# HiLab-git/FPL-plus

Hardware: AMD Instinct MI355X
Metric: 3D volumes/sec (train step, 80x160x160) (higher is better)
Workload: dtype bf16; 1 GPU; UNet3D-DSBN 32-base-ch bf16 (fp32 master weights), per-GPU batch 2x1x80x160x160 synthetic VS crops, DiceLoss + Adam, domain alternating per step; global_batch=2, parallelism=dp1, step=zero_grad+forward+loss+backward+allreduce+adam

## Files before the change

fpl-plus_amd/csrc/common.h:

```cpp
#pragma once
#include <hip/hip_runtime.h>
#include <math.h>
#include <stdint.h>
#include <stdio.h>
#include <stdarg.h>
#include <string.h>
#include "../../include/fplx.h"

typedef __bf16 bf16_t;

#define FPLX_WAVE 64

inline char* fplx_err_buf() {
  static thread_local char buf[512];
  return buf;
}
inline int fplx_fail(int code, const char* fmt, ...) {
  va_list ap;
  va_start(ap, fmt);
  vsnprintf(fplx_err_buf(), 512, fmt, ap);
  va_end(ap);
  return code;
}
inline int fplx_check_launch(const char* what) {
// ... 221 lines not shown
  t.step = (gridDim.x - c + 7u) >> 3;
  return t;
}
template <typename... P, typename... A>
inline void fplx_launch(void (*kernel)(P...), dim3 grid, dim3 block, size_t lds, hipStream_t st, A... args) {
  if (lds) (void)hipFuncSetAttribute((const void*)kernel, hipFuncAttributeMaxDynamicSharedMemorySize, (int)lds);
  kernel<<<grid, block, lds, st>>>(args...);
}
#endif
#define FPLX_KNOB_LIST(X)                                                                                              \
  X(XCD, "xcd", 1)                                                    \
  X(BRICK, "brick", 1)                                    \
  X(BRICK_FILL, "brick_fill", 192)           \
  X(BRICK_GEO, "brick_geo", -1)                    \
  X(BRICK_KSPLIT, "brick_ksplit", 0)                                             \
  X(EDGE_BLOCKS, "edge_blocks", 1024)                             \
  X(STEM_ROWS, "stem_rows", 1)                                              \
  X(OUTCONV_T, "outconv_t", 1)                                 \
  X(OUTCONV_DGRAD_MFMA, "outconv_dgrad_mfma", 1)                                                                       \
  X(OUTCONV_FWD_ROWS, "outconv_fwd_rows", 1)  \
  X(OUTCONV_DGRAD_ROWS, "outconv_dgrad_rows", 1)  \
  X(PACK_TILED, "pack_tiled", 1)                                                                                       \
  X(PACK_MULTI, "pack_multi", 1)                                                                                       \
  X(MARCH, "march", 1)                           \
  X(MARCH64_FW, "march64_fw", 0)                                \
  X(MARCH_DS, "march_ds", 0)                                       \
  X(MARCH128, "march128", 1)                                                                                           \
  X(MARCH64_LW, "march64_lw", 1)            \
  X(MARCH32_V2, "march32_v2", 4)              \
  X(WG_COT_MINVOX, "wg_cot_minvox", 0)                                                                                 \
  X(WG_TW, "wg_tw", 0)                                                                                                 \
  X(WG_CIT, "wg_cit", 2)                                                                                               \
  X(WG_COT, "wg_cot", 2)                                                                                               \
  X(WG_DS, "wg_ds", 0)                                                                                                 \
  X(WG_VOX, "wg_vox", 1)                              \
  X(WG_ROLL, "wg_roll", 1)                     \
  X(WG_ROLL_GEO, "wg_roll_geo", 0)          \
  X(WG_ROLL_M16, "wg_roll_m16", 1)                 \
  X(WG_ROLL_MB, "wg_roll_mb", 1)            \
  X(WG_ROLL_CUS, "wg_roll_cus", 256)                                \
  X(WG_ROLL_OVH, "wg_roll_ovh", 9)                     \
  X(WG_ROLL_MINVOX, "wg_roll_minvox", 0)                                                   \
  X(WG_ROLL2D, "wg_roll2d", 1)              \
  X(WG_ROLL2D_OVH, "wg_roll2d_ovh", 3)      \
  X(WG_REDUCE_ROWS, "wg_reduce_rows", 8)    \
  X(WG_VOX_LW, "wg_vox_lw", 1)              \
  X(WG_VOX_CUS, "wg_vox_cus", 128)          \
  X(WG_VOX_MAXV, "wg_vox_maxv", 10000)         \
  X(TILE_NT, "tile_nt", 0)                                                                                             \
  X(TILE_KS, "tile_ks", 0)                                                                                             \
  X(MID_TILE, "mid_tile", 1)                                                                                           \
  X(DECONV_ROWS, "deconv_rows", 1)                                                                                     \
  X(DECONV_DGRAD_ROWS, "deconv_dgrad_rows", 1)   \
  X(ROWS_SMALL_DIV, "rows_small_div", 16)   \
  X(EW_GROUP, "ew_group", 1)                                                                                           \
  X(POOL_COL, "pool_col", 1)                         \
  X(EW_INFLIGHT, "ew_inflight", 2)          \
  X(EW_INFLIGHT_REDUCE, "ew_inflight_reduce", 2)
enum FplxKnobId {
#define FPLX_KNOB_ENUM(id, key, def) FPLX_K_##id,
  FPLX_KNOB_LIST(FPLX_KNOB_ENUM)
#undef FPLX_KNOB_ENUM
  FPLX_K_COUNT
};
extern "C" __attribute__((visibility("hidden"))) int64_t fplx_knob_values[FPLX_K_COUNT];
static inline int64_t fplx_knob(int id) { return __atomic_load_n(&fplx_knob_values[id], __ATOMIC_RELAXED); }
static inline int fplx_xcd_on() { return (int)fplx_knob(FPLX_K_XCD); }

static inline int fplx_rows_for(int64_t voxels) {
  constexpr int cap = 512;
  const int div = voxels <= 32768 ? (int)fplx_knob(FPLX_K_ROWS_SMALL_DIV) : 64;
  int64_t r = (voxels + div - 1) / div;
  if (r > cap) r = cap;
  if (r < 1) r = 1;
  return (int)r;
}
```

fpl-plus_amd/csrc/conv_generic.hip:

```cpp
#include "internal.h"

namespace {

struct Strides { int64_t n, d, h, w, c; };

constexpr int CO_T = 8;
constexpr int FWD_THREADS = 256;
constexpr int MAX_ROWS = 2048;

template <typename TX, typename TW, typename TY>
__global__ void __launch_bounds__(FWD_THREADS)
conv_fwd_generic(const TX* __restrict__ x, Strides xs, const TW* __restrict__ wp, const float* __restrict__ bias,
                 TY* __restrict__ y, Strides ys, int N, int D, int H, int W, int Cin, int Cout,
                 int KD, int KH, int KW, float* __restrict__ stats, int64_t tiles) {
  const int co0 = blockIdx.y * CO_T;
  const int64_t V = (int64_t)N * D * H * W;
  float s[CO_T], q[CO_T];
#pragma unroll
  for (int j = 0; j < CO_T; ++j) s[j] = q[j] = 0.f;
  const int pd = KD / 2, ph = KH / 2, pw = KW / 2;
  for (int64_t tile = blockIdx.x; tile < tiles; tile += gridDim.x) {
    const int64_t v = tile * FWD_THREADS + threadIdx.x;
    const bool valid = v < V;
    int64_t r = valid ? v : 0;
// ... 1214 lines not shown
  Strides xs{(int64_t)d * h * w * ldx, (int64_t)h * w * ldx, (int64_t)w * ldx, ldx, 1};
  Strides ys{(int64_t)4 * sd * d * h * w * ldy, (int64_t)(sd == 2 ? 4 : 2) * h * w * ldy, (int64_t)2 * w * ldy, ldy, 1};
  bool done = false;
  if (dt == FPLX_BF16) {
    const size_t m = fplx_mfma_deconv2_wgrad_ws_bytes(n, d, h, w, cin, cout);
    if (m > 0) {
      int r = fplx_mfma_deconv2_wgrad(x, ldx, dy, ldy, dw, db, n, d, h, w, cin, cout, ws, m, sd, st);
      if (r < 0) return r;
      if (r == 1) { done = true; used = m; db = nullptr; }
    }
  }
  float* bpart = (float*)((char*)ws + used);
  if (done) {
  } else if (dt == FPLX_F32)
    wgrad_generic<float, float, true><<<grid, WG_THREADS, 0, st>>>((const float*)x, xs, (const float*)dy, ys, part, n,
                                                                   d, h, w, cin, cout, sd, 2, 2, chunks);
  else if (dt == FPLX_BF16)
    wgrad_generic<bf16_t, bf16_t, true><<<grid, WG_THREADS, 0, st>>>((const bf16_t*)x, xs, (const bf16_t*)dy, ys, part,
                                                                     n, d, h, w, cin, cout, sd, 2, 2, chunks);
  else
    return fplx_fail(FPLX_E_BADDTYPE, "deconv2_wgrad: dtype %d", dt);
  if (!done) wgrad_reduce<<<grid_for((int64_t)taps * cout * cin, 256, 1024), 256, 0, st>>>(part, dw, chunks, taps, cout, cin, 1);
  if (db) {
    Strides yb{(int64_t)4 * sd * d * h * w * ldy, (int64_t)4 * h * w * ldy, (int64_t)2 * w * ldy, ldy, 1};
    if (dt == FPLX_F32) launch_bias_grad<float>((const float*)dy, yb, n, sd * d, 2 * h, 2 * w, cout, bpart, db, st);
    else launch_bias_grad<bf16_t>((const bf16_t*)dy, yb, n, sd * d, 2 * h, 2 * w, cout, bpart, db, st);
  }
  return fplx_check_launch("deconv2_wgrad");
}

int fplx_deconv2_fwd(const void* x, int64_t ldx, const void* wf, const float* bias, void* y, int64_t ldy, int n, int d,
                     int h, int w, int cin, int cout, int dt, fplx_stream_t stream) {
  return deconv_fwd_impl(x, ldx, wf, bias, y, ldy, n, d, h, w, cin, cout, dt, 2, stream);
}
int fplx_deconv2_dgrad(const void* dy, int64_t ldy, const void* wb, void* dx, int64_t ldx, int n, int d, int h, int w,
                       int cin, int cout, int dt, fplx_stream_t stream) {
  return deconv_dgrad_impl(dy, ldy, wb, dx, ldx, n, d, h, w, cin, cout, dt, 2, stream);
}
size_t fplx_deconv2_wgrad_ws_bytes(int n, int d, int h, int w, int cin, int cout) {
  return deconv_wgrad_ws_impl(n, d, h, w, cin, cout, 2);
}
int fplx_deconv2_wgrad(const void* x, int64_t ldx, const void* dy, int64_t ldy, float* dw, float* db, int n, int d,
                       int h, int w, int cin, int cout, int dt, void* ws, size_t ws_bytes, fplx_stream_t stream) {
  return deconv_wgrad_impl(x, ldx, dy, ldy, dw, db, n, d, h, w, cin, cout, dt, ws, ws_bytes, 2, stream);
}
int fplx_deconv122_fwd(const void* x, int64_t ldx, const void* wf, const float* bias, void* y, int64_t ldy, int n, int d,
                       int h, int w, int cin, int cout, int dt, fplx_stream_t stream) {
  return deconv_fwd_impl(x, ldx, wf, bias, y, ldy, n, d, h, w, cin, cout, dt, 1, stream);
}
int fplx_deconv122_dgrad(const void* dy, int64_t ldy, const void* wb, void* dx, int64_t ldx, int n, int d, int h, int w,
                         int cin, int cout, int dt, fplx_stream_t stream) {
  return deconv_dgrad_impl(dy, ldy, wb, dx, ldx, n, d, h, w, cin, cout, dt, 1, stream);
}
size_t fplx_deconv122_wgrad_ws_bytes(int n, int d, int h, int w, int cin, int cout) {
  return deconv_wgrad_ws_impl(n, d, h, w, cin, cout, 1);
}
int fplx_deconv122_wgrad(const void* x, int64_t ldx, const void* dy, int64_t ldy, float* dw, float* db, int n, int d,
                         int h, int w, int cin, int cout, int dt, void* ws, size_t ws_bytes, fplx_stream_t stream) {
  return deconv_wgrad_impl(x, ldx, dy, ldy, dw, db, n, d, h, w, cin, cout, dt, ws, ws_bytes, 1, stream);
}

}
```

fpl-plus_amd/csrc/conv_mfma.hip:

```cpp
#include "internal.h"
#include "gfx950.h"
#include <stdlib.h>

namespace {

constexpr int DIRECT_THREADS = 256;

template <int MT, int NTL, int MODE>
__global__ void __launch_bounds__(DIRECT_THREADS)
conv_fwd_direct(const bf16_t* __restrict__ x, int64_t ldx, const bf16_t* __restrict__ wp,
                const float* __restrict__ bias, bf16_t* __restrict__ y, int64_t ldy, int N, int D, int H, int W,
                int Cin, int Cout, float* __restrict__ stats, float* __restrict__ partial = nullptr) {
  const int lane = threadIdx.x & 63, wave = threadIdx.x >> 6;
  const int r = lane & 31, kh8 = (lane >> 5) * 8;
  const int64_t V = (int64_t)N * D * H * W;
  const int64_t m0 = ((int64_t)blockIdx.x * 4 + wave) * (MT * 32);
  const int n0 = blockIdx.y * (NTL * 32);

  int vn[MT], vd[MT], vh[MT], vw[MT];
  bool vok[MT];
#pragma unroll
  for (int t = 0; t < MT; ++t) {
    int64_t v = m0 + t * 32 + r;
    vok[t] = v < V;
// ... 1198 lines not shown
    __syncthreads();
    if (tid < 32) {
      const int cc = tid >> 3, j = tid & 7;
      float t = 0.f;
      for (int k = 0; k < 64; ++k) t += red[(k * 4 + cc) * 8 + j];
      bpart[(int64_t)blockIdx.x * Cout + cot * 32 + tid] = t;
    }
  }
}

__global__ void __launch_bounds__(64) deconv_bias_reduce(const float* __restrict__ bpart, int rows, int C, float* __restrict__ db) {
  const int c = blockIdx.x;
  float t = 0.f;
  for (int r = threadIdx.x; r < rows; r += 64) t += bpart[(int64_t)r * C + c];
  t = wave_sum(t);
  if (threadIdx.x == 0) db[c] = t;
}

__global__ void __launch_bounds__(256)
deconv_wgrad_reduce(const float* __restrict__ part, int nblk, int npairs, int cit, int Cin, int Cout,
                    float* __restrict__ dw, int ntaps) {
  __shared__ float red[256];
  const int64_t per = (int64_t)8 * cit * 1024, total = npairs * per;
  const int64_t i = (int64_t)blockIdx.x * 64 + (threadIdx.x & 63);
  const int pl = threadIdx.x >> 6, o = threadIdx.x & 63;
  float t = 0.f;
  if (i < total)
    for (int b = pl; b < nblk; b += 4) t += part[(int64_t)b * total + i];
  red[pl * 64 + o] = t;
  __syncthreads();
  if (pl != 0 || i >= total) return;
  t = red[o] + red[64 + o] + red[128 + o] + red[192 + o];
  const int co_l = i & 31, ci_l = (i >> 5) & 31, c = (int)((i >> 10) % cit), tap = (int)((i / (1024 * cit)) % 8);
  const int pair = (int)(i / per);
  const int ncig = Cin / (32 * cit);
  const int co = (pair / ncig) * 32 + co_l, ci = ((pair % ncig) * cit + c) * 32 + ci_l;
  if (tap < ntaps) dw[((int64_t)ci * Cout + co) * ntaps + tap] = t;
}

struct DwCfg { int cit, npairs, nblk; size_t ws; };
inline DwCfg dw_cfg(int n, int d, int h, int w, int cin, int cout) {
  DwCfg c;
  c.cit = (cin % 128 == 0) ? 4 : (cin % 64 == 0 ? 2 : 1);
  c.npairs = (cin / (32 * c.cit)) * (cout / 32);
  const int64_t chunks = ((int64_t)n * d * h * w + 127) / 128;
  int nb = 512 / c.npairs;
  if (nb < 1) nb = 1;
  if (nb > chunks) nb = (int)chunks;
  c.nblk = nb;
  c.ws = (size_t)c.nblk * c.npairs * 8 * c.cit * 1024 * sizeof(float) + (size_t)c.nblk * cout * sizeof(float);
  return c;
}

template <int NT, int KC>
__global__ void __launch_bounds__(256, 2)
conv_fwd_tile(const bf16_t* __restrict__ x, int64_t ldx, const bf16_t* __restrict__ wp, const float* __restrict__ bias,
              bf16_t* __restrict__ y, int64_t ldy, int N, int D, int H, int W, int Cin, int Cout,
              float* __restrict__ stats, float* __restrict__ partial, int tap_lo, int tap_cnt, int xcd) {
  constexpr int MTL = 128, THREADS = MTL * 2, NTW = NT / 64;
  constexpr int ROWB = KC * 2, CH = KC / 8, RP = THREADS / CH;
  constexpr int PA = MTL / RP, PB = NT / RP;
  constexpr int KS = KC / 16;
  constexpr int A_BYTES = MTL * ROWB, B_BYTES = NT * ROWB, BUF = A_BYTES + B_BYTES;
  extern __shared__ __attribute__((aligned(16))) char smem[];
  const int tid = threadIdx.x, lane = tid & 63, wave = tid >> 6;
  const int r = lane & 31, khalf = lane >> 5;
  const int wm = wave >> 1, wn = wave & 1;
  const int64_t V = (int64_t)N * D * H * W;
  const FplxBlock bid = fplx_xcd_block(xcd);
  const int64_t m0 = (int64_t)bid.x * MTL;
  const int n0 = bid.y * NT;
  const int c16 = tid % CH, row0 = tid / CH;
  const bf16_t* abase[PA];
  uint32_t amask[PA];
#pragma unroll
  for (int u = 0; u < PA; ++u) {
    int64_t v = m0 + row0 + RP * u;
    const bool ok = v < V;
    if (!ok) v = 0;
    abase[u] = x + v * ldx + c16 * 8;
    unsigned q = (unsigned)v;
    const int ww0 = (int)(q % (unsigned)W); q /= (unsigned)W;
    const int hh0 = (int)(q % (unsigned)H); q /= (unsigned)H;
    const int dd0 = (int)(q % (unsigned)D);
    uint32_t m = 0;
    for (int t = 0; t < 27; ++t) {
      const int dd = dd0 + t / 9 - 1, hh = hh0 + (t / 3) % 3 - 1, ww = ww0 + t % 3 - 1;
      if (ok && dd >= 0 && dd < D && hh >= 0 && hh < H && ww >= 0 && ww < W) m |= 1u << t;
    }
    amask[u] = m;
  }
  const int nkc = Cin / KC;
  const int ntaps = (tap_cnt - bid.z + (int)gridDim.z - 1) / (int)gridDim.z;
  const int niter = ntaps * nkc;
  auto swz = [](int row) { return (row / (16 / CH)) % CH; };
  uint4 areg00, areg01, areg02, areg03, breg00, breg01, breg02, breg03;
  uint4 areg10, areg11, areg12, areg13, breg10, breg11, breg12, breg13;
  areg02 = areg03 = breg01 = breg02 = breg03 = make_uint4(0, 0, 0, 0);
  areg12 = areg13 = breg11 = breg12 = breg13 = make_uint4(0, 0, 0, 0);
  unsigned zmask0 = 0, zmask1 = 0;
#define TILE_A(U, S)                                                                                                \
  if (PA > (U)) {                                                                                                   \
    constexpr int u_ = (U) < PA ? (U) : 0;                                                                          \
    const bool in_ = (amask[u_] >> tap_) & 1u;                                                                      \
    zmask##S |= in_ ? 0u : (1u << (U));                                                                             \
    areg##S##U = *reinterpret_cast<const uint4*>(abase[u_] + (in_ ? aoff_ : (int64_t)kc_));                         \
// ... 644 lines not shown
      int rc = fplx_check_launch("mfma_deconv2_fwd_rows");
      return rc < 0 ? rc : 1;
    }
  }
  dim3 grid((unsigned)((V + 127) / 128), cout / 32, sd);
  deconv_fwd_mfma<<<grid, DIRECT_THREADS, 0, st>>>((const bf16_t*)x, ldx, (const bf16_t*)wf, bias, (bf16_t*)y, ldy, n, d,
                                                   h, w, cin, cout, sd, vec_ok, fplx_xcd_on());
  int rc = fplx_check_launch("mfma_deconv2_fwd");
  return rc < 0 ? rc : 1;
}

extern "C" int fplx_mfma_deconv2_dgrad(const void* dy, int64_t ldy, const void* wb, void* dx, int64_t ldx, int n, int d,
                                       int h, int w, int cin, int cout, int sd, hipStream_t st) {
  if (cout % 16 != 0 || cin % 32 != 0 || ldy % 8 != 0 || ((uintptr_t)dy % 16) || ((uintptr_t)wb % 16)) return 0;
  const int64_t V = (int64_t)n * d * h * w;
  if (V * 8 >= ((int64_t)1 << 31)) return 0;
  if (sd == 2 && fplx_knob(FPLX_K_DECONV_DGRAD_ROWS) && V >= 16 * 1024 && ldx % 8 == 0 && ((uintptr_t)dx % 16) == 0 &&
      ((cout == 32 && cin == 64) || (cout == 64 && cin == 128))) {
    const int mb = cin == 64 ? 64 : 32;
    const int segsW = (w + mb - 1) / mb;
    const int64_t nseg = (int64_t)n * d * h * segsW;
    const unsigned nb = (unsigned)(nseg < 512 ? nseg : 512);
    if (cout == 32)
      deconv_dgrad_rows<1, 2><<<nb, 256, 0, st>>>((const bf16_t*)dy, ldy, (const bf16_t*)wb, (bf16_t*)dx, ldx, n, d, h, w, segsW, nseg, fplx_xcd_on());
    else
      deconv_dgrad_rows<2, 4><<<nb, 256, 0, st>>>((const bf16_t*)dy, ldy, (const bf16_t*)wb, (bf16_t*)dx, ldx, n, d, h, w, segsW, nseg, fplx_xcd_on());
    int rcr = fplx_check_launch("mfma_deconv2_dgrad_rows");
    return rcr < 0 ? rcr : 1;
  }
  if (sd == 2 && fplx_knob(FPLX_K_DECONV_DGRAD_ROWS) && ((V + 127) / 128) * (cin / 64) < 128 && cin % 64 == 0 && cout % 16 == 0 &&
      ldx % 8 == 0 && ((uintptr_t)dx % 16) == 0) {
    dim3 gs((unsigned)((V + 31) / 32), cin / 64);
    deconv_dgrad_small<<<gs, 256, 0, st>>>((const bf16_t*)dy, ldy, (const bf16_t*)wb, (bf16_t*)dx, ldx, n, d, h, w, cout, cin);
    int rcs = fplx_check_launch("mfma_deconv2_dgrad_small");
    return rcs < 0 ? rcs : 1;
  }
  const bool wide = cin % 64 == 0;
  const dim3 grid = wide ? dim3((unsigned)((V + 255) / 256), cin / 64) : dim3((unsigned)((V + 511) / 512), cin / 32);
  const bool deep = wide && (int64_t)grid.x * grid.y < 192;
  const auto k = deep ? (sd == 2 ? conv_fwd_direct<1, 2, 1> : conv_fwd_direct<1, 2, 2>)
                 : wide ? (sd == 2 ? conv_fwd_direct<2, 2, 1> : conv_fwd_direct<2, 2, 2>)
                        : (sd == 2 ? conv_fwd_direct<4, 1, 1> : conv_fwd_direct<4, 1, 2>);
  fplx_launch(k, deep ? dim3((unsigned)((V + 127) / 128), cin / 64) : grid, DIRECT_THREADS, 0, st, (const bf16_t*)dy, ldy,
              (const bf16_t*)wb, nullptr, (bf16_t*)dx, ldx, n, d, h, w, cout, cin, nullptr, nullptr);
  int rc = fplx_check_launch("mfma_deconv2_dgrad");
  return rc < 0 ? rc : 1;
}

extern "C" size_t fplx_mfma_deconv2_wgrad_ws_bytes(int n, int d, int h, int w, int cin, int cout) {
  if (cin % 32 != 0 || cout % 32 != 0) return 0;
  return dw_cfg(n, d, h, w, cin, cout).ws;
}

extern "C" int fplx_mfma_deconv2_wgrad(const void* x, int64_t ldx, const void* dy, int64_t ldy, float* dw, float* db,
                                       int n, int d, int h, int w, int cin, int cout, void* ws, size_t ws_bytes,
                                       int sd, hipStream_t st) {
  if (cin % 32 != 0 || cout % 32 != 0 || ldx % 8 != 0 || ldy % 8 != 0 || ((uintptr_t)x % 16) || ((uintptr_t)dy % 16))
    return 0;
  const DwCfg c = dw_cfg(n, d, h, w, cin, cout);
  if (ws_bytes < c.ws) return fplx_fail(FPLX_E_WORKSPACE, "mfma_deconv2_wgrad: workspace %zu < %zu", ws_bytes, c.ws);
  const size_t lds = (size_t)(c.cit + 8) * 128 * 64;
  float* bpart = db ? (float*)((char*)ws + (size_t)c.nblk * c.npairs * 8 * c.cit * 1024 * sizeof(float)) : nullptr;
  auto launch = [&](auto kernel) {
    fplx_launch(kernel, dim3(c.nblk, c.npairs), 256, lds, st, (const bf16_t*)x, ldx, (const bf16_t*)dy, ldy, (float*)ws, bpart, n, d,
                h, w, cin, cout, sd);
  };
  if (c.cit == 4) launch(deconv_wgrad_mfma<4>);
  else if (c.cit == 2) launch(deconv_wgrad_mfma<2>);
  else launch(deconv_wgrad_mfma<1>);
  const int64_t total = (int64_t)c.npairs * 8 * c.cit * 1024;
  if (db) deconv_bias_reduce<<<cout, 64, 0, st>>>(bpart, c.nblk, cout, db);
  deconv_wgrad_reduce<<<(unsigned)((total + 63) / 64), 256, 0, st>>>((const float*)ws, c.nblk, c.npairs, c.cit, cin, cout, dw,
                                                                      4 * sd);
  int rc = fplx_check_launch("mfma_deconv2_wgrad");
  return rc < 0 ? rc : 1;
}
```

fpl-plus_amd/csrc/internal.h:

```cpp
#pragma once
#include "common.h"

extern "C" {

int fplx_march_ok(int n, int d, int h, int w, int cin, int cout);
int fplx_march_rows(int n, int d, int h, int w, int cin, int cout);
int fplx_march_variant(int n, int d, int h, int w, int cin, int cout);
int fplx_march_conv3d_fwd(const void* x, int64_t ldx, const void* wp, const float* bias, void* y, int64_t ldy, int n, int d,
                          int h, int w, int cin, int cout, float* stats, hipStream_t st, const void* x1, void* y1, int twod);
int fplx_march_conv3d_fwd_act(const void* x, int64_t ldx, const void* wp, const float* bias, void* y, int64_t ldy, int n,
                              int d, int h, int w, int cin, int cout, float* stats, hipStream_t st, const void* x1, void* y1,
                              int twod, const float* slope, int nmod0);

int fplx_brick_ok(int n, int d, int h, int w, int cin, int cout);
int fplx_brick_first(int n, int d, int h, int w, int cin, int cout);
int fplx_brick_plan(int n, int d, int h, int w, int cin, int cout, int* geo, int* ksplit, int* bricks);
int fplx_brick_conv3d_fwd_act(const void* x, int64_t ldx, const void* wp, const float* bias, void* y, int64_t ldy, int n,
                              int d, int h, int w, int cin, int cout, float* stats, float* partial, int geo, int ksplit,
                              hipStream_t st, const float* slope, const void* x1, int nmod0);

int fplx_wgroll_ok(int n, int d, int h, int w, int cin, int cout, int mid, int splitx);
size_t fplx_wgroll_ws_bytes(int n, int d, int h, int w, int cin, int cout);
int fplx_wgroll_conv3d_wgrad(const void* x, int64_t ldx, const void* dy, int64_t ldy, float* dw, int n, int d, int h, int w,
                             int cin, int cout, void* ws, size_t ws_bytes, hipStream_t st, const void* x1, int mid);

int fplx_mfma_conv3d_plan(int n, int d, int h, int w, int cin, int cout, int mid, int* kernel, int* geo, int* ksplit);
int fplx_mfma_conv3d_stats_rows(int n, int d, int h, int w, int cin, int cout, int mid);
size_t fplx_mfma_conv3d_fwd_ws_bytes(int n, int d, int h, int w, int cin, int cout, int mid);
int fplx_mfma_conv3d_fwd(const void* x, int64_t ldx, const void* wp, const float* bias, void* y, int64_t ldy, int n, int d,
                         int h, int w, int cin, int cout, float* stats, void* ws, size_t ws_bytes, int mid, hipStream_t st);
int fplx_mfma_conv3d_act_ok(int n, int d, int h, int w, int cin, int cout, int mid);
int fplx_mfma_conv3d_act_cat2_ok(int n, int d, int h, int w, int cin, int cout, int mid);
int fplx_mfma_conv3d_fwd_act(const void* x, int64_t ldx, const void* wp, const float* bias, const float* slope, void* y,
                             int64_t ldy, int n, int d, int h, int w, int cin, int cout, void* ws, size_t ws_bytes, int mid,
                             hipStream_t st);
int fplx_mfma_conv3d_fwd_act_cat2(const void* x0, const void* x1, int64_t ldx, const void* wp, const float* bias,
                                  const float* slope, void* y, int64_t ldy, int n, int d, int h, int w, int cin, int cout,
                                  int nmod0, hipStream_t st);
int fplx_mfma_conv3d_wgrad_cit(int n, int d, int h, int w, int cin, int cout);
size_t fplx_mfma_conv3d_wgrad_ws_bytes(int n, int d, int h, int w, int cin, int cout);
int fplx_mfma_conv3d_wgrad(const void* x, int64_t ldx, const void* dy, int64_t ldy, float* dw, int n, int d, int h, int w,
                           int cin, int cout, void* ws, size_t ws_bytes, hipStream_t st, const void* x1, int mid);
int fplx_wgrad_reduce_launch(const float* part, int nblk, int npairs, int cin, int cout, float* dw, int mid, hipStream_t st);
int fplx_mfma_deconv2_fwd(const void* x, int64_t ldx, const void* wf, const float* bias, void* y, int64_t ldy, int n, int d,
                          int h, int w, int cin, int cout, int sd, hipStream_t st);
int fplx_mfma_deconv2_dgrad(const void* dy, int64_t ldy, const void* wb, void* dx, int64_t ldx, int n, int d, int h, int w,
                            int cin, int cout, int sd, hipStream_t st);
size_t fplx_mfma_deconv2_wgrad_ws_bytes(int n, int d, int h, int w, int cin, int cout);
int fplx_mfma_deconv2_wgrad(const void* x, int64_t ldx, const void* dy, int64_t ldy, float* dw, float* db, int n, int d,
                            int h, int w, int cin, int cout, void* ws, size_t ws_bytes, int sd, hipStream_t st);

int fplx_edge_stem_rows(int n, int d, int h, int w, int cin, int cout);
int fplx_edge_stem_fwd(const float* x, const void* wf, const float* bias, void* y, int64_t ldy, int n, int d, int h, int w,
                       int cin, int cout, float* stats, hipStream_t st);
size_t fplx_edge_stem_wgrad_ws_bytes(int n, int d, int h, int w, int cin, int cout);
int fplx_edge_stem_wgrad(const float* x, const void* dy, int64_t ldy, float* dw, int n, int d, int h, int w, int cin,
                         int cout, void* ws, hipStream_t st);
int fplx_edge_stem_wgrad_bn(const float* x, const void* dy, int64_t ldy, float* dw, int n, int d, int h, int w, int cin,
                            int cout, void* ws, hipStream_t st, const void* y, int64_t ldyy, const float* mean,
                            const float* rstd, const float* scale, const float* shift, const float* slope, const float* coef);
int fplx_edge_outconv_fwd(const void* x, int64_t ldx, const float* wf, const float* bias, float* out, int n, int d, int h,
                          int w, int cin, int ncls, hipStream_t st);
int fplx_edge_outconv_dgrad(const float* dl, const void* wb, void* dx, int64_t ldx, int n, int d, int h, int w, int c0,
                            int ncls, hipStream_t st);
size_t fplx_edge_outconv_wgrad_ws_bytes(int n, int d, int h, int w, int c0, int ncls);
int fplx_edge_outconv_wgrad(const void* x, int64_t ldx, const float* dl, float* dw, int n, int d, int h, int w, int c0,
                            int ncls, void* ws, hipStream_t st);
int fplx_edge_outconv_bn_ok(int n, int d, int h, int w, int c0, int ncls);
int fplx_edge_outconv_bn_rows(int n, int d, int h, int w, int ncls);
int fplx_edge_outconv_fwd_bn(const void* y, int64_t ldy, const float* scale, const float* shift, const float* slope, void* a,
                             int64_t lda, const float* wf, const float* bias, float* out, int n, int d, int h, int w, int c0,
                             int ncls, hipStream_t st);
int fplx_edge_outconv_dgrad_bn(int mode, const float* dl, const void* wb, const void* y, int64_t ldy, const float* mean,
                               const float* rstd, const float* scale, const float* shift, const float* slope,
                               const float* coef, float* part, void* dy, int64_t lddy, int n, int d, int h, int w, int c0,
                               int ncls, hipStream_t st);
size_t fplx_edge_outconv_wgrad_bn_ws_bytes(int n, int d, int h, int w, int c0, int ncls);
int fplx_edge_outconv_wgrad_bn(const void* y, int64_t ldy, const float* scale, const float* shift, const float* slope,
                               const float* dl, float* dw, float* db, int n, int d, int h, int w, int c0, int ncls, void* ws,
                               hipStream_t st);

}
```

fpl-plus_amd/fplx/ops.py:

```python
import ctypes
import math

import numpy as np
import torch
from . import _lib
from ._lib import F32, BF16, call

_DT = {torch.float32: F32, torch.bfloat16: BF16}


def dt_of(t):
    try:
        return _DT[t.dtype]
    except KeyError:
        raise ValueError("fplx: unsupported activation dtype {0:}".format(t.dtype))


def ptr(t):
    return 0 if t is None else t.data_ptr()


def stream():
    return torch.cuda.current_stream().cuda_stream

# ... 159 lines not shown
    call("fplx_conv2d_fwd_cat2" if mid else "fplx_conv3d_fwd_cat2", ptr(x0), ptr(x1), ld_of(x0), ptr(wp), ptr(bias), ptr(y), ld_of(y), n, d, h, w, cin,
         cout, ptr(stats), stream())


def conv3d_dgrad_split2(dy, wb, dx0, dx1, dims, cin, cout, mid=False):
    n, d, h, w = dims
    assert ld_of(dx0) == ld_of(dx1)
    call("fplx_conv2d_dgrad_split2" if mid else "fplx_conv3d_dgrad_split2", ptr(dy), ld_of(dy), ptr(wb), ptr(dx0), ptr(dx1), ld_of(dx0), n, d, h, w, cin,
         cout, stream())


def conv3d_wgrad_cat2(x0, x1, dy, dw, dims, cin, cout, ws, mid=False):
    n, d, h, w = dims
    assert ld_of(x0) == ld_of(x1)
    call("fplx_conv2d_wgrad_cat2" if mid else "fplx_conv3d_wgrad_cat2", ptr(x0), ptr(x1), ld_of(x0), ptr(dy), ld_of(dy),
         ptr(dw), n, d, h, w, cin, cout, ptr(ws), ws.numel() * ws.element_size(), stream())


def conv3d_fwd_act_ok(dims, cin, cout, mid=False, cat2=False):
    n, d, h, w = dims
    return _lib.lib().fplx_conv3d_fwd_act_ok(n, d, h, w, cin, cout, 1 if mid else 0, 1 if cat2 else 0) == 1


def conv3d_fwd_act(x0, x1, wp, bias, slope, y, dims, cin, cout, mid=False, n_x0=0):
    n, d, h, w = dims
    ws = _fwd_scratch(conv3d_fwd_ws_bytes(dims, cin, cout, (3, 3, 3), BF16, BF16, mid), y.device)
    if x1 is not None:
        assert ld_of(x0) == ld_of(x1)
    call("fplx_conv3d_fwd_act", ptr(x0), ptr(x1), ld_of(x0), ptr(wp), ptr(bias), ptr(slope), ptr(y), ld_of(y), n, d, h, w, cin,
         cout, 1 if mid else 0, int(n_x0), ptr(ws), 0 if ws is None else ws.numel(), stream())


def _dc(sd):
    return "fplx_deconv2_" if sd == 2 else "fplx_deconv122_"


def deconv2_fwd(x, wf, bias, y, dims, cin, cout, sd=2):
    n, d, h, w = dims
    call(_dc(sd) + "fwd", ptr(x), ld_of(x), ptr(wf), ptr(bias), ptr(y), ld_of(y), n, d, h, w, cin, cout,
         dt_of(x), stream())


def deconv2_dgrad(dy, wb, dx, dims, cin, cout, sd=2):
    n, d, h, w = dims
    call(_dc(sd) + "dgrad", ptr(dy), ld_of(dy), ptr(wb), ptr(dx), ld_of(dx), n, d, h, w, cin, cout,
         dt_of(dy), stream())


def deconv2_wgrad_ws_bytes(dims, cin, cout, sd=2):
    n, d, h, w = dims
    return getattr(_lib.lib(), _dc(sd) + "wgrad_ws_bytes")(n, d, h, w, cin, cout)


def deconv2_wgrad(x, dy, dw, db, dims, cin, cout, ws, sd=2):
    n, d, h, w = dims
    call(_dc(sd) + "wgrad", ptr(x), ld_of(x), ptr(dy), ld_of(dy), ptr(dw), ptr(db), n, d, h, w, cin, cout,
         dt_of(x), ptr(ws), ws.numel() * ws.element_size(), stream())


def upsample2_fwd(x, y, dims, c, sd=2):
    n, d, h, w = dims
    call("fplx_upsample2_fwd", ptr(x), ld_of(x), ptr(y), ld_of(y), n, d, h, w, c, dt_of(x), sd, stream())


def upsample2_bwd(dy, dx, dims, c, sd=2):
    n, d, h, w = dims
    call("fplx_upsample2_bwd", ptr(dy), ld_of(dy), ptr(dx), ld_of(dx), n, d, h, w, c, dt_of(dy), sd, stream())


def bn_train_finalize(stats, rows, c, count, gamma, beta, rm, rv, nbt, bnbuf, momentum=0.1, eps=1e-5):
    call("fplx_bn_train_finalize", ptr(stats), rows, c, count, ptr(gamma), ptr(beta), ptr(rm), ptr(rv), ptr(nbt),
         momentum, eps, ptr(bnbuf[0]), ptr(bnbuf[1]), ptr(bnbuf[2]), ptr(bnbuf[3]), stream())


def bn_eval_prepare(gamma, beta, rm, rv, bnbuf, eps=1e-5):
    c = gamma.numel()
    call("fplx_bn_eval_prepare", ptr(gamma), ptr(beta), ptr(rm), ptr(rv), eps, c, ptr(bnbuf[2]), ptr(bnbuf[3]),
         stream())


def bn_act_fwd(y, out, bnbuf, slope, p, seed, sid, c):
    call("fplx_bn_act_fwd", ptr(y), ld_of(y), ptr(out), ld_of(out), ptr(bnbuf[2]), ptr(bnbuf[3]), ptr(slope),
         float(p), int(seed), int(sid), y.shape[0], c, dt_of(y), stream())


def num_partials(voxels):
    return _lib.lib().fplx_num_partials(voxels)


def outconv_bn_rows(dims, c0=32, ncls=2):
    n, d, h, w = dims
    return _lib.lib().fplx_outconv_bn_rows(n, d, h, w, int(c0), int(ncls))


def outconv_bn_ok(dims, c0, ncls):
    return outconv_bn_rows(dims, c0, ncls) > 0


def outconv_fwd_bn(y, bnbuf, slope, a, wf, bias, logits, dims, c0, ncls):
    n, d, h, w = dims
    call("fplx_outconv_fwd_bn", ptr(y), ld_of(y), ptr(bnbuf[2]), ptr(bnbuf[3]), ptr(slope), ptr(a), int(c0) if a is None else ld_of(a),
         ptr(wf), ptr(bias), ptr(logits), n, d, h, w, int(c0), int(ncls), stream())


def outconv_wgrad_bn_ws_bytes(dims, c0, ncls):
    n, d, h, w = dims
# ... 1152 lines not shown
```

include/fplx.h:

```cpp
#ifndef FPLX_H
#define FPLX_H

#include <stddef.h>
#include <stdint.h>

#ifdef __cplusplus
extern "C" {
#endif
#pragma GCC visibility push(default)

typedef void* fplx_stream_t;

enum { FPLX_F32 = 0, FPLX_BF16 = 1 };

enum {
  FPLX_OK = 0,
  FPLX_E_BADSHAPE = -1,
  FPLX_E_BADDTYPE = -2,
  FPLX_E_WORKSPACE = -3,
  FPLX_E_HIP = -4,
  FPLX_E_NULL = -5
};

int fplx_version(void);
// ... 9 lines not shown
int fplx_tuning_key(int index, char* buf, size_t n);
int fplx_conv3d_plan_query(int n, int d, int h, int w, int cin, int cout, int kd, int kh, int kw, int x_dt, int y_dt,
                           int* kernel, int* geometry, int* ksplit, int* stats_rows);

int fplx_pack_conv_weight(const float* w, void* wf, void* wb, int cout, int cin, int kd, int kh, int kw,
                          int dt, fplx_stream_t stream);
int fplx_pack_conv_weights_batched(int n, const float* const* w, void* const* wf, void* const* wb, const int* cout,
                                   const int* cin, int dt, float* const* stamp, int verify, fplx_stream_t stream);
int fplx_pack_weights_multi(int n, const int* kind, const float* const* w, void* const* wf, void* const* wb, const int* a,
                            const int* b, const int* taps, const int* dt, fplx_stream_t stream);
int fplx_pack_deconv_weight(const float* w, void* wf, void* wb, int cin, int cout, int dt,
                            fplx_stream_t stream);

int fplx_conv3d_stats_rows(int n, int d, int h, int w, int cin, int cout, int kd, int kh, int kw, int x_dt, int y_dt);
size_t fplx_conv3d_fwd_ws_bytes(int n, int d, int h, int w, int cin, int cout, int kd, int kh, int kw, int x_dt, int y_dt);
int fplx_conv3d_fwd(const void* x, int x_dt, int64_t sn, int64_t sd, int64_t sh, int64_t sw, int64_t sc,
                    const void* wp, const float* bias,
                    void* y, int y_dt, int64_t yn, int64_t yd, int64_t yh, int64_t yw, int64_t yc,
                    int n, int d, int h, int w, int cin, int cout, int kd, int kh, int kw,
                    float* stats, void* ws, size_t ws_bytes, fplx_stream_t stream);

size_t fplx_conv3d_wgrad_ws_bytes(int n, int d, int h, int w, int cin, int cout, int kd, int kh, int kw);
int fplx_conv3d_wgrad(const void* x, int x_dt, int64_t sn, int64_t sd, int64_t sh, int64_t sw, int64_t sc,
                      const void* dy, int dy_dt, int64_t yn, int64_t yd, int64_t yh, int64_t yw, int64_t yc,
                      float* dw, float* db, int n, int d, int h, int w, int cin, int cout,
                      int kd, int kh, int kw, void* ws, size_t ws_bytes, fplx_stream_t stream);

int fplx_stem_wgrad_bn(const float* x, const void* y, int64_t ldy, const void* dout, int64_t ldd, const float* mean,
                       const float* rstd, const float* scale, const float* shift, const float* slope, const float* coef,
                       float* dw, int n, int d, int h, int w, int cin, int cout, void* ws, size_t ws_bytes, fplx_stream_t stream);

int fplx_conv3d_cat2_ok(int n, int d, int h, int w, int cin, int cout);
int fplx_conv3d_fwd_cat2(const void* x0, const void* x1, int64_t ldx, const void* wp, const float* bias, void* y,
                         int64_t ldy, int n, int d, int h, int w, int cin, int cout, float* stats,
                         fplx_stream_t stream);
int fplx_conv3d_dgrad_split2(const void* dy, int64_t ldy, const void* wb, void* dx0, void* dx1, int64_t ldx, int n,
                             int d, int h, int w, int cin, int cout, fplx_stream_t stream);
int fplx_conv3d_wgrad_cat2(const void* x0, const void* x1, int64_t ldx, const void* dy, int64_t ldy, float* dw, int n,
                           int d, int h, int w, int cin, int cout, void* ws, size_t ws_bytes, fplx_stream_t stream);

int fplx_conv3d_fwd_act_ok(int n, int d, int h, int w, int cin, int cout, int mid, int cat2);
int fplx_conv3d_fwd_act(const void* x0, const void* x1, int64_t ldx, const void* wp, const float* bias,
                        const float* prelu_slope, void* y, int64_t ldy, int n, int d, int h, int w, int cin, int cout,
                        int mid, int n_x0, void* ws, size_t ws_bytes, fplx_stream_t stream);

int fplx_deconv2_fwd(const void* x, int64_t ldx, const void* wf, const float* bias, void* y, int64_t ldy,
                     int n, int d, int h, int w, int cin, int cout, int dt, fplx_stream_t stream);
int fplx_deconv2_dgrad(const void* dy, int64_t ldy, const void* wb, void* dx, int64_t ldx,
                       int n, int d, int h, int w, int cin, int cout, int dt, fplx_stream_t stream);
size_t fplx_deconv2_wgrad_ws_bytes(int n, int d, int h, int w, int cin, int cout);
int fplx_deconv2_wgrad(const void* x, int64_t ldx, const void* dy, int64_t ldy, float* dw, float* db,
                       int n, int d, int h, int w, int cin, int cout, int dt,
                       void* ws, size_t ws_bytes, fplx_stream_t stream);

int fplx_pack_conv2d_weight(const float* w, void* wf, void* wb, int cout, int cin, int dt, fplx_stream_t stream);
int fplx_conv2d_stats_rows(int n, int d, int h, int w, int cin, int cout, int x_dt, int y_dt);
size_t fplx_conv2d_fwd_ws_bytes(int n, int d, int h, int w, int cin, int cout, int x_dt, int y_dt);
int fplx_conv2d_fwd(const void* x, int x_dt, int64_t sn, int64_t sd, int64_t sh, int64_t sw, int64_t sc,
                    const void* wp, const float* bias, void* y, int y_dt, int64_t yn, int64_t yd, int64_t yh,
                    int64_t yw, int64_t yc, int n, int d, int h, int w, int cin, int cout,
                    float* stats, void* ws, size_t ws_bytes, fplx_stream_t stream);
int fplx_conv2d_fwd_cat2(const void* x0, const void* x1, int64_t ldx, const void* wp, const float* bias, void* y,
                         int64_t ldy, int n, int d, int h, int w, int cin, int cout, float* stats,
                         fplx_stream_t stream);
int fplx_conv2d_dgrad_split2(const void* dy, int64_t ldy, const void* wb, void* dx0, void* dx1, int64_t ldx, int n,
                             int d, int h, int w, int cin, int cout, fplx_stream_t stream);
size_t fplx_conv2d_wgrad_ws_bytes(int n, int d, int h, int w, int cin, int cout);
int fplx_conv2d_wgrad(const void* x, int x_dt, int64_t sn, int64_t sd, int64_t sh, int64_t sw, int64_t sc,
                      const void* dy, int dy_dt, int64_t yn, int64_t yd, int64_t yh, int64_t yw, int64_t yc,
                      float* dw, float* db, int n, int d, int h, int w, int cin, int cout,
                      void* ws, size_t ws_bytes, fplx_stream_t stream);
int fplx_conv2d_wgrad_cat2(const void* x0, const void* x1, int64_t ldx, const void* dy, int64_t ldy, float* dw, int n,
                           int d, int h, int w, int cin, int cout, void* ws, size_t ws_bytes, fplx_stream_t stream);
int fplx_maxpool122_fwd(const void* x, int64_t ldx, void* y, int64_t ldy, int n, int d, int h, int w, int c,
                        int dt, fplx_stream_t stream);
int fplx_maxpool122_bwd(const void* x, int64_t ldx, const void* dy, int64_t ldy, const void* dskip, int64_t lds,
                        void* dx, int64_t ldo, int n, int d, int h, int w, int c, int dt, fplx_stream_t stream);
int fplx_pack_deconv122_weight(const float* w, void* wf, void* wb, int cin, int cout, int dt, fplx_stream_t stream);
int fplx_deconv122_fwd(const void* x, int64_t ldx, const void* wf, const float* bias, void* y, int64_t ldy,
                       int n, int d, int h, int w, int cin, int cout, int dt, fplx_stream_t stream);
int fplx_deconv122_dgrad(const void* dy, int64_t ldy, const void* wb, void* dx, int64_t ldx,
                         int n, int d, int h, int w, int cin, int cout, int dt, fplx_stream_t stream);
size_t fplx_deconv122_wgrad_ws_bytes(int n, int d, int h, int w, int cin, int cout);
int fplx_deconv122_wgrad(const void* x, int64_t ldx, const void* dy, int64_t ldy, float* dw, float* db,
                         int n, int d, int h, int w, int cin, int cout, int dt,
                         void* ws, size_t ws_bytes, fplx_stream_t stream);

int fplx_bn_train_finalize(const float* stats, int rows, int c, int64_t count,
                           const float* gamma, const float* beta, float* running_mean, float* running_var,
                           int64_t* num_batches_tracked, float momentum, float eps,
                           float* mean, float* rstd, float* scale, float* shift, fplx_stream_t stream);
int fplx_channel_stats(const void* x, int64_t ldx, int64_t voxels, int c, int dt, float* stats,
                       fplx_stream_t stream);
int fplx_bn_eval_prepare(const float* gamma, const float* beta, const float* running_mean,
                         const float* running_var, float eps, int c, float* scale, float* shift,
                         fplx_stream_t stream);
int fplx_bn_act_fwd(const void* y, int64_t ldy, void* out, int64_t ldo, const float* scale, const float* shift,
                    const float* slope, float p, uint64_t seed, uint32_t stream_id,
                    int64_t voxels, int c, int dt, fplx_stream_t stream);
int fplx_bn_act_bwd_reduce(const void* y, int64_t ldy, const void* dout, int64_t ldd,
                           const float* mean, const float* rstd, const float* scale, const float* shift,
                           const float* slope, float p, uint64_t seed, uint32_t stream_id,
                           int64_t voxels, int c, int dt, float* part, fplx_stream_t stream);
int fplx_bn_act_bwd_finalize(const float* part, int rows, int c, int64_t count, int train,
                             float* dgamma, float* dbeta, float* dslope, float* coef, fplx_stream_t stream);
int fplx_bn_act_bwd_apply(const void* y, int64_t ldy, const void* dout, int64_t ldd, void* dy, int64_t ldo,
// ... 245 lines not shown
```

Before: 252.2 volumes/s.

## Add cost-model planner and range-split MFMA kernel for deconv weight gradient

Adds a cost model that chooses the input-channel tile width and the number of voxel ranges for the transposed-conv weight gradient. It weighs HBM and L2 traffic, serial chunk-chain latency and the cost of reducing partials. A new MFMA kernel handles contiguous chunk ranges with register prefetch of the next chunk. A separate finish kernel then reduces the per-range partials, splitting the reduction into slices when there are many ranges. This replaces the fixed dw_cfg heuristic by default, aiming at better occupancy and less partial traffic, at the cost of an extra launch and tuning constants that may not fit every shape.

```diff
diff --git a/fpl-plus_amd/csrc/common.h b/fpl-plus_amd/csrc/common.h
--- a/fpl-plus_amd/csrc/common.h
+++ b/fpl-plus_amd/csrc/common.h
@@ -297,6 +297,9 @@
   X(MID_TILE, "mid_tile", 1)                                                                                           \
   X(DECONV_ROWS, "deconv_rows", 1)                                                                                     \
   X(DECONV_DGRAD_ROWS, "deconv_dgrad_rows", 1)   \
+  X(DECONV_WGRAD_PLAN, "deconv_wgrad_plan", 1)   \
+  X(DECONV_WGRAD_CIT, "deconv_wgrad_cit", 0)     \
+  X(DECONV_WGRAD_RANGES, "deconv_wgrad_ranges", 0)  \
   X(ROWS_SMALL_DIV, "rows_small_div", 16)   \
   X(EW_GROUP, "ew_group", 1)                                                                                           \
   X(POOL_COL, "pool_col", 1)                         \
diff --git a/fpl-plus_amd/csrc/conv_generic.hip b/fpl-plus_amd/csrc/conv_generic.hip
--- a/fpl-plus_amd/csrc/conv_generic.hip
+++ b/fpl-plus_amd/csrc/conv_generic.hip
@@ -1290,6 +1290,22 @@
                          int cin, int cout, int dt, fplx_stream_t stream) {
   return deconv_dgrad_impl(dy, ldy, wb, dx, ldx, n, d, h, w, cin, cout, dt, 1, stream);
 }
+int fplx_deconv2_wgrad_plan_query(int n, int d, int h, int w, int cin, int cout, int sd, int* ci_tiles, int* pairs, int* ranges,
+                                  int* chunks_per_range, size_t* partial_bytes, size_t* bias_bytes, int64_t* bounds,
+                                  int bounds_cap) {
+  FPLX_REQUIRE(n > 0 && d > 0 && h > 0 && w > 0 && cin > 0 && cout > 0 && (sd == 1 || sd == 2), FPLX_E_BADSHAPE,
+               "deconv2_wgrad_plan_query: bad shape");
+  int c = 0, p = 0, r = 0, k = 0;
+  size_t pb = 0, bb = 0;
+  if (!fplx_mfma_deconv2_wgrad_plan(n, d, h, w, cin, cout, sd, &c, &p, &r, &k, &pb, &bb, bounds, bounds_cap)) c = p = r = k = 0;
+  if (ci_tiles) *ci_tiles = c;
+  if (pairs) *pairs = p;
+  if (ranges) *ranges = r;
+  if (chunks_per_range) *chunks_per_range = k;
+  if (partial_bytes) *partial_bytes = pb;
+  if (bias_bytes) *bias_bytes = bb;
+  return FPLX_OK;
+}
 size_t fplx_deconv122_wgrad_ws_bytes(int n, int d, int h, int w, int cin, int cout) {
   return deconv_wgrad_ws_impl(n, d, h, w, cin, cout, 1);
 }
diff --git a/fpl-plus_amd/csrc/conv_mfma.hip b/fpl-plus_amd/csrc/conv_mfma.hip
--- a/fpl-plus_amd/csrc/conv_mfma.hip
+++ b/fpl-plus_amd/csrc/conv_mfma.hip
@@ -1274,6 +1274,232 @@
   return c;
 }
 
+__host__ __device__ inline int64_t dw_range_lo(int64_t chunks, int r, int R) { return chunks * r / R; }
+
+template <int CIT>
+__global__ void __launch_bounds__(256)
+deconv_wgrad_mfma_rng(const bf16_t* __restrict__ x, int64_t ldx, const bf16_t* __restrict__ dy, int64_t ldy,
+                      float* __restrict__ part, float* __restrict__ bpart, int N, int D, int H, int W, int Cin, int Cout,
+                      int sd) {
+  constexpr int KV = 128;
+  extern __shared__ __attribute__((aligned(16))) char smem[];
+  char* xs = smem;
+  char* dys = smem + CIT * KV * 64;
+  const int tid = threadIdx.x, lane = tid & 63;
+  const int wave = __builtin_amdgcn_readfirstlane(tid >> 6);
+  const int ncig = Cin / (32 * CIT);
+  const int cot = blockIdx.y / ncig, cig = blockIdx.y % ncig;
+  const int64_t V = (int64_t)N * D * H * W;
+  const int64_t chunks = (V + KV - 1) / KV;
+  const int64_t c0 = dw_range_lo(chunks, blockIdx.x, gridDim.x), c1 = dw_range_lo(chunks, blockIdx.x + 1, gridDim.x);
+  const int g = lane >> 4, q = (lane & 15) >> 2, p = lane & 3;
+  const int lane_off = (8 * (g >> 1) + q) * 64 + (16 * (g & 1) + 4 * p) * 2;
+  const int c16 = tid & 3, vx0 = tid >> 2;
+  const bool want_bias = bpart != nullptr && cig == 0;
+  const bool small = V <= 0x7fffffff;
+  float bsum[8];
+#pragma unroll
+  for (int j = 0; j < 8; ++j) bsum[j] = 0.f;
+  f32x16 acc[2][CIT];
+#pragma unroll
+  for (int t = 0; t < 2; ++t)
+#pragma unroll
+    for (int c = 0; c < CIT; ++c)
+#pragma unroll
+      for (int i = 0; i < 16; ++i) acc[t][c][i] = 0.f;
+  uint4 xv[2][CIT], gv[2][8];
+  auto fetch = [&](int64_t ch) {
+#pragma unroll
+    for (int half = 0; half < 2; ++half) {
+      int64_t vv = ch * KV + vx0 + 64 * half;
+#pragma unroll
+      for (int c = 0; c < CIT; ++c) xv[half][c] = make_uint4(0, 0, 0, 0);
+#pragma unroll
+      for (int tap = 0; tap < 8; ++tap) gv[half][tap] = make_uint4(0, 0, 0, 0);
+      if (vv < V) {
+#pragma unroll
+        for (int c = 0; c < CIT; ++c)
+          xv[half][c] = *reinterpret_cast<const uint4*>(x + vv * ldx + (cig * CIT + c) * 32 + c16 * 8);
+        int w0, h0, d0;
+        int64_t n0;
+        if (small) {
+          unsigned u = (unsigned)vv;
+          w0 = (int)(u % (unsigned)W); u /= (unsigned)W;
+          h0 = (int)(u % (unsigned)H); u /= (unsigned)H;
+          d0 = (int)(u % (unsigned)D); n0 = u / (unsigned)D;
+        } else {
+          w0 = (int)(vv % W); vv /= W;
+          h0 = (int)(vv % H); vv /= H;
+          d0 = (int)(vv % D); n0 = vv / D;
+        }
+        const int64_t obase = ((n0 * sd * D + sd * d0) * 2 * H + 2 * h0) * 2 * W + 2 * w0;
+#pragma unroll
+        for (int tap = 0; tap < 8; ++tap) {
+          if (tap < 4 * sd) {
+            const int64_t ov = obase + ((int64_t)(tap >> 2) * 2 * H + ((tap >> 1) & 1)) * 2 * W + (tap & 1);
+            gv[half][tap] = *reinterpret_cast<const uint4*>(dy + ov * ldy + cot * 32 + c16 * 8);
+          }
+        }
+      }
+    }
+  };
+  if (c0 < c1) fetch(c0);
+  for (int64_t ch = c0; ch < c1; ++ch) {
+#pragma unroll
+    for (int half = 0; half < 2; ++half) {
+      const int vox = vx0 + 64 * half;
+#pragma unroll
+      for (int c = 0; c < CIT; ++c) *reinterpret_cast<uint4*>(xs + (c * KV + vox) * 64 + c16 * 16) = xv[half][c];
+#pragma unroll
+      for (int tap = 0; tap < 8; ++tap) {
+        *reinterpret_cast<uint4*>(dys + (tap * KV + vox) * 64 + c16 * 16) = gv[half][tap];
+        if (want_bias) {
+          const bf16x8 b8 = *reinterpret_cast<const bf16x8*>(&gv[half][tap]);
+#pragma unroll
+          for (int j = 0; j < 8; ++j) bsum[j] += (float)b8[j];
+        }
+      }
+    }
+    __syncthreads();
+    if (ch + 1 < c1) fetch(ch + 1);
+    for (int ks = 0; ks < KV / 16; ++ks) {
+      bf16x8 bfr[2];
+#pragma unroll
+      for (int t = 0; t < 2; ++t) bfr[t] = tr_frag(dys + ((2 * wave + t) * KV + ks * 16) * 64 + lane_off);
+#pragma unroll
+      for (int c = 0; c < CIT; ++c) {
+        const bf16x8 afr = tr_frag(xs + (c * KV + ks * 16) * 64 + lane_off);
+#pragma unroll
+        for (int t = 0; t < 2; ++t) acc[t][c] = __builtin_amdgcn_mfma_f32_32x32x16_bf16(afr, bfr[t], acc[t][c], 0, 0, 0);
+      }
+    }
+    __syncthreads();
+  }
+  float* out = part + ((int64_t)blockIdx.x * gridDim.y + blockIdx.y) * (8 * CIT * 1024);
+  const int co = lane & 31, rbase = (lane >> 5) * 4;
+#pragma unroll
+  for (int t = 0; t < 2; ++t)
+#pragma unroll
+    for (int c = 0; c < CIT; ++c)
+#pragma unroll
+      for (int i = 0; i < 16; ++i) {
+        const int ci = (i & 3) + 8 * (i >> 2) + rbase;
+        out[(((2 * wave + t) * CIT + c) * 32 + ci) * 32 + co] = acc[t][c][i];
+      }
+  if (want_bias) {
+    float* red = reinterpret_cast<float*>(smem);
+#pragma unroll
+    for (int j = 0; j < 8; ++j) red[tid * 8 + j] = bsum[j];
+    __syncthreads();
+    if (tid < 32) {
+      const int cc = tid >> 3, j = tid & 7;
+      float t = 0.f;
+      for (int k = 0; k < 64; ++k) t += red[(k * 4 + cc) * 8 + j];
+      bpart[(int64_t)blockIdx.x * Cout + cot * 32 + tid] = t;
+    }
+  }
+}
+
+template <int NT, int SLOTS>
+__global__ void __launch_bounds__(32 * SLOTS)
+deconv_wgrad_finish(const float* __restrict__ part, const float* __restrict__ bpart, int R, int npairs, int cit, int Cin,
+                    int Cout, float* __restrict__ dw, float* __restrict__ db, int S, int vec) {
+  __shared__ float red[SLOTS][32][NT + 1];
+  const int co_l = threadIdx.x & 31, slot = threadIdx.x >> 5;
+  const int ci = blockIdx.x * (SLOTS / S) + slot / S, slice = slot % S, cot = blockIdx.y;
+  const int ncig = Cin / (32 * cit);
+  const int64_t per = (int64_t)8 * cit * 1024, rstride = npairs * per, tstride = (int64_t)cit * 1024;
+  const float* base = part + (int64_t)(cot * ncig + ci / (32 * cit)) * per + (((ci >> 5) % cit) * 32 + (ci & 31)) * 32 + co_l;
+  const int co = cot * 32 + co_l;
+  const bool bias = db != nullptr && ci == 0;
+  const int r0 = (int)dw_range_lo(R, slice, S), r1 = (int)dw_range_lo(R, slice + 1, S);
+  float a[NT + 1];
+#pragma unroll
+  for (int t = 0; t <= NT; ++t) a[t] = 0.f;
+  for (int r = r0; r < r1; r += 8) {
+    float v[8][NT + 1];
+#pragma unroll
+    for (int u = 0; u < 8; ++u) {
+      const bool ok = r + u < r1;
+#pragma unroll
+      for (int t = 0; t < NT; ++t) v[u][t] = ok ? base[(int64_t)(r + u) * rstride + t * tstride] : 0.f;
+      v[u][NT] = ok && bias ? bpart[(int64_t)(r + u) * Cout + co] : 0.f;
+    }
+#pragma unroll
+    for (int u = 0; u < 8; ++u)
+#pragma unroll
+      for (int t = 0; t <= NT; ++t) a[t] += v[u][t];
+  }
+  if (S > 1) {
+#pragma unroll
+    for (int t = 0; t <= NT; ++t) red[slot][co_l][t] = a[t];
+    __syncthreads();
+    if (slice != 0) return;
+    for (int s = 1; s < S; ++s)
+#pragma unroll
+      for (int t = 0; t <= NT; ++t) a[t] += red[slot + s][co_l][t];
+  }
+  float* o = dw + ((int64_t)ci * Cout + co) * NT;
+  if (vec) {
+#pragma unroll
+    for (int t = 0; t < NT; t += 4) *reinterpret_cast<float4*>(o + t) = make_float4(a[t], a[t + 1], a[t + 2], a[t + 3]);
+  } else {
+#pragma unroll
+    for (int t = 0; t < NT; ++t) o[t] = a[t];
+  }
+  if (bias) db[co] = a[NT];
+}
+
+constexpr double DW_HBM = 5.0e6, DW_L2 = 6.0e6, DW_PART_W = 4.0e6, DW_PART_R = 4.0e6;
+constexpr double DW_T0 = 3.0, DW_T0CIT = 0.5, DW_TCHUNK = 2.4, DW_TCIT = 0.2, DW_TFIN0 = 3.0, DW_TFIN = 0.5;
+struct DwPlan { int cit, npairs, ranges, cpr, slices; size_t part_bytes; };
+inline int dw_slices(int ranges) {
+  int s = 1;
+  while (s < 32 && s * 8 < ranges) s *= 2;
+  return s;
+}
+inline DwPlan dw_plan(int n, int d, int h, int w, int cin, int cout, int sd) {
+  const int64_t V = (int64_t)n * d * h * w, chunks = (V + 127) / 128;
+  const int force_cit = (int)fplx_knob(FPLX_K_DECONV_WGRAD_CIT), force_r = (int)fplx_knob(FPLX_K_DECONV_WGRAD_RANGES);
+  const double tiles = (double)(cin / 32) * (cout / 32);
+  DwPlan cand[36];
+  double cost_of[36], best_cost = 0;
+  int ncand = 0;
+  for (int cit = 4; cit >= 1; cit >>= 1) {
+    if ((cin / 32) % cit != 0 || (force_cit > 0 && force_cit != cit && (cin / 32) % force_cit == 0)) continue;
+    const int ncig = cin / (32 * cit), npairs = ncig * (cout / 32);
+    int64_t rmax = 512 / npairs;
+    if (rmax < 1) rmax = 1;
+    if (rmax > chunks) rmax = chunks;
+    for (int64_t r = 1;; r *= 2) {
+      int R = (int)(r < rmax ? r : rmax);
+      if (force_r > 0) R = (int)(force_r < rmax ? force_r : rmax);
+      const int cpr = (int)((chunks + R - 1) / R), S = dw_slices(R);
+      const double unique = (double)V * 2 * (cin + 4.0 * sd * cout);
+      const double reread = (double)V * 2 * (cin * (double)(cout / 32) + 4.0 * sd * cout * ncig) - unique;
+      const double partial = (double)R * tiles * 32768.0;
+      const double occ = cit == 4 ? 256.0 : 512.0;
+      const double rounds = (double)(int64_t)(((double)R * npairs + occ - 1) / occ);
+      const double t_bytes = unique / DW_HBM + reread / DW_L2;
+      const double t_chain = rounds * (DW_T0 + DW_T0CIT * cit + cpr * (DW_TCHUNK + DW_TCIT * cit)) + partial / DW_PART_W;
+      const double t_fin = DW_TFIN0 + partial / DW_PART_R + (double)((R / S + 7) / 8) * DW_TFIN;
+      const double cost = (t_bytes > t_chain ? t_bytes : t_chain) + t_fin;
+      if (ncand == 0 || cost < best_cost) best_cost = cost;
+      cost_of[ncand] = cost;
+      cand[ncand++] = DwPlan{cit, npairs, R, cpr, S, (size_t)R * npairs * 8 * cit * 1024 * sizeof(float)};
+      if (force_r > 0 || r >= rmax || ncand == 36) break;
+    }
+  }
+  int best = 0;
+  for (int i = 1; i < ncand; ++i) {
+    if (cost_of[i] > 1.1 * best_cost) continue;
+    if (cost_of[best] > 1.1 * best_cost || cand[i].part_bytes < cand[best].part_bytes ||
+        (cand[i].part_bytes == cand[best].part_bytes && cost_of[i] < cost_of[best]))
+      best = i;
+  }
+  return cand[best];
+}
+
 template <int NT, int KC>
 __global__ void __launch_bounds__(256, 2)
 conv_fwd_tile(const bf16_t* __restrict__ x, int64_t ldx, const bf16_t* __restrict__ wp, const float* __restrict__ bias,
@@ -2024,6 +2250,29 @@
   return dw_cfg(n, d, h, w, cin, cout).ws;
 }
 
+extern "C" int fplx_mfma_deconv2_wgrad_plan(int n, int d, int h, int w, int cin, int cout, int sd, int* cit, int* pairs,
+                                            int* ranges, int* cpr, size_t* part_bytes, size_t* bias_bytes, int64_t* bounds, int cap) {
+  if (cin % 32 != 0 || cout % 32 != 0) return 0;
+  const int64_t chunks = ((int64_t)n * d * h * w + 127) / 128;
+  DwPlan p;
+  if (fplx_knob(FPLX_K_DECONV_WGRAD_PLAN)) {
+    p = dw_plan(n, d, h, w, cin, cout, sd);
+    if (bounds && cap > p.ranges)
+      for (int r = 0; r <= p.ranges; ++r) bounds[r] = dw_range_lo(chunks, r, p.ranges);
+  } else {
+    const DwCfg c = dw_cfg(n, d, h, w, cin, cout);
+    p = DwPlan{c.cit, c.npairs, c.nblk, (int)((chunks + c.nblk - 1) / c.nblk), 0,
+               (size_t)c.nblk * c.npairs * 8 * c.cit * 1024 * sizeof(float)};
+  }
+  if (cit) *cit = p.cit;
+  if (pairs) *pairs = p.npairs;
+  if (ranges) *ranges = p.ranges;
+  if (cpr) *cpr = p.cpr;
+  if (part_bytes) *part_bytes = p.part_bytes;
+  if (bias_bytes) *bias_bytes = (size_t)p.ranges * cout * sizeof(float);
+  return 1;
+}
+
 extern "C" int fplx_mfma_deconv2_wgrad(const void* x, int64_t ldx, const void* dy, int64_t ldy, float* dw, float* db,
                                        int n, int d, int h, int w, int cin, int cout, void* ws, size_t ws_bytes,
                                        int sd, hipStream_t st) {
@@ -2031,6 +2280,28 @@
     return 0;
   const DwCfg c = dw_cfg(n, d, h, w, cin, cout);
   if (ws_bytes < c.ws) return fplx_fail(FPLX_E_WORKSPACE, "mfma_deconv2_wgrad: workspace %zu < %zu", ws_bytes, c.ws);
+  if (fplx_knob(FPLX_K_DECONV_WGRAD_PLAN)) {
+    const DwPlan p = dw_plan(n, d, h, w, cin, cout, sd);
+    if (p.part_bytes + (size_t)p.ranges * cout * sizeof(float) > c.ws)
+      return fplx_fail(FPLX_E_WORKSPACE, "mfma_deconv2_wgrad: the plan's partials exceed the workspace bound");
+    float* bp = db ? (float*)((char*)ws + p.part_bytes) : nullptr;
+    auto launch = [&](auto kernel) {
+      fplx_launch(kernel, dim3(p.ranges, p.npairs), 256, (size_t)(p.cit + 8) * 128 * 64, st, (const bf16_t*)x, ldx, (const bf16_t*)dy, ldy,
+                  (float*)ws, bp, n, d, h, w, cin, cout, sd);
+    };
+    if (p.cit == 4) launch(deconv_wgrad_mfma_rng<4>);
+    else if (p.cit == 2) launch(deconv_wgrad_mfma_rng<2>);
+    else launch(deconv_wgrad_mfma_rng<1>);
+    const int slots = p.slices > 8 ? 32 : 8, vec = ((uintptr_t)dw % 16) == 0;
+    const dim3 fg(cin / (slots / p.slices), cout / 32);
+    auto finish = [&](auto kernel) {
+      kernel<<<fg, 32 * slots, 0, st>>>((const float*)ws, bp, p.ranges, p.npairs, p.cit, cin, cout, dw, db, p.slices, vec);
+    };
+    if (sd == 2) { if (slots == 32) finish(deconv_wgrad_finish<8, 32>); else finish(deconv_wgrad_finish<8, 8>); }
+    else { if (slots == 32) finish(deconv_wgrad_finish<4, 32>); else finish(deconv_wgrad_finish<4, 8>); }
+    int rcp = fplx_check_launch("mfma_deconv2_wgrad");
+    return rcp < 0 ? rcp : 1;
+  }
   const size_t lds = (size_t)(c.cit + 8) * 128 * 64;
   float* bpart = db ? (float*)((char*)ws + (size_t)c.nblk * c.npairs * 8 * c.cit * 1024 * sizeof(float)) : nullptr;
   auto launch = [&](auto kernel) {
diff --git a/fpl-plus_amd/csrc/internal.h b/fpl-plus_amd/csrc/internal.h
--- a/fpl-plus_amd/csrc/internal.h
+++ b/fpl-plus_amd/csrc/internal.h
@@ -47,6 +47,8 @@
 int fplx_mfma_deconv2_dgrad(const void* dy, int64_t ldy, const void* wb, void* dx, int64_t ldx, int n, int d, int h, int w,
                             int cin, int cout, int sd, hipStream_t st);
 size_t fplx_mfma_deconv2_wgrad_ws_bytes(int n, int d, int h, int w, int cin, int cout);
+int fplx_mfma_deconv2_wgrad_plan(int n, int d, int h, int w, int cin, int cout, int sd, int* cit, int* pairs, int* ranges,
+                                 int* cpr, size_t* part_bytes, size_t* bias_bytes, int64_t* bounds, int cap);
 int fplx_mfma_deconv2_wgrad(const void* x, int64_t ldx, const void* dy, int64_t ldy, float* dw, float* db, int n, int d,
                             int h, int w, int cin, int cout, void* ws, size_t ws_bytes, int sd, hipStream_t st);
 
diff --git a/fpl-plus_amd/fplx/ops.py b/fpl-plus_amd/fplx/ops.py
--- a/fpl-plus_amd/fplx/ops.py
+++ b/fpl-plus_amd/fplx/ops.py
@@ -235,6 +235,18 @@
     return getattr(_lib.lib(), _dc(sd) + "wgrad_ws_bytes")(n, d, h, w, cin, cout)
 
 
+def deconv2_wgrad_plan(dims, cin, cout, sd=2):
+    n, d, h, w = dims
+    i4 = [ctypes.c_int() for _ in range(4)]
+    sz = [ctypes.c_size_t() for _ in range(2)]
+    bounds = (ctypes.c_int64 * 514)(*([-1] * 514))
+    _lib.check(_lib.lib().fplx_deconv2_wgrad_plan_query(n, d, h, w, int(cin), int(cout), int(sd), *[ctypes.byref(v) for v in i4 + sz],
+                                                        bounds, 514))
+    r = i4[2].value
+    return dict(ci_tiles=i4[0].value, pairs=i4[1].value, ranges=r, chunks_per_range=i4[3].value, partial_bytes=sz[0].value,
+                bias_bytes=sz[1].value, bounds=list(bounds[:r + 1]) if r and bounds[0] >= 0 else None)
+
+
 def deconv2_wgrad(x, dy, dw, db, dims, cin, cout, ws, sd=2):
     n, d, h, w = dims
     call(_dc(sd) + "wgrad", ptr(x), ld_of(x), ptr(dy), ld_of(dy), ptr(dw), ptr(db), n, d, h, w, cin, cout,
diff --git a/include/fplx.h b/include/fplx.h
--- a/include/fplx.h
+++ b/include/fplx.h
@@ -85,6 +85,9 @@
 int fplx_deconv2_wgrad(const void* x, int64_t ldx, const void* dy, int64_t ldy, float* dw, float* db,
                        int n, int d, int h, int w, int cin, int cout, int dt,
                        void* ws, size_t ws_bytes, fplx_stream_t stream);
+int fplx_deconv2_wgrad_plan_query(int n, int d, int h, int w, int cin, int cout, int sd, int* ci_tiles, int* pairs,
+                                  int* ranges, int* chunks_per_range, size_t* partial_bytes, size_t* bias_bytes,
+                                  int64_t* bounds, int bounds_cap);
 
 int fplx_pack_conv2d_weight(const float* w, void* wf, void* wb, int cout, int cin, int dt, fplx_stream_t stream);
 int fplx_conv2d_stats_rows(int n, int d, int h, int w, int cin, int cout, int x_dt, int y_dt);
```

Measured after the change: 253.3 volumes/s (median of 6 runs). Within noise of the previous version (+0.4%).
